# Vchitect/Latte

Measured on AMD Instinct MI355X. Metric: denoising steps/sec, higher is better.
Workload: dtype f16; 1 GPU; Latte-XL/2 FaceForensics (uncond) 16x256x256 -> latents 16x4x32x32, DDIM on the '250' respacing, random-init weights; per_gpu_batch=8, global_batch=8, parallelism=dp1 (independent samples)

## Files before the change

include/latte_amd_debug.h:

```cpp
#ifndef LATTE_AMD_DEBUG_H_
#define LATTE_AMD_DEBUG_H_
#include <stdint.h>
#ifdef __cplusplus
extern "C" {
#endif

int latte_debug_gemm(const void* A, const void* W, const float* bias, void* out, const float* gate, int M, int N,
                     int K, int gate_stride, int rows_per_sample, int epi, int dtype, int variant, void* stream);
int latte_debug_gemm_gelu(const void* A, const void* W, const float* bias, void* out, void* aux, int M, int N, int K, int epi, int dtype,
                          void* stream);
int latte_debug_gemm_lo8(const void* A, const void* W, const void* A8, const void* W8, const float* bias, void* out, const float* gate,
                         int M, int N, int K, int gate_stride, int rows_per_sample, int epi, int dtype, void* stream);
int latte_debug_pack_w8(const void* w, void* out8, int64_t n, int dtype, void* stream);
int latte_debug_pack_w4(const void* w, void* out4, void* out_scale, int N, int K, int dtype, void* stream);
int latte_debug_ln_modulate_split4(const float* x, void* y, void* y4, void* y4s, const float* shift, const float* scale, int mod_stride, int M,
                                   int D, int rows_per_sample, int dtype, void* stream);
int latte_debug_gemm_lo4(const void* A, const void* W, const void* A4, const void* A4s, const void* W4, const void* W4s, const float* bias,
                         void* out, const float* gate, int M, int N, int K, int gate_stride, int rows_per_sample, int epi, int dtype,
                         void* stream);
int latte_debug_ln_modulate_split8(const float* x, void* y, void* y8, const float* shift, const float* scale, int mod_stride, int M, int D,
                                   int rows_per_sample, int dtype, void* stream);
int latte_debug_qkv_attention_split8(const void* xn, const void* w, const float* bias, void* out, void* out8, int B, int F, int T, int D,
                                     int heads, int mode, int dtype, void* stream);
int latte_debug_gemm_choice(int M, int N, int K, int epi);
int latte_debug_qkv_attention_fusable(int D, int heads, int F, int T, int mode, int64_t rows);
int latte_debug_gemm_tn_plan(int M, int N, int K, int* rows_per_split);
int latte_debug_attention(const void* qkv, void* out, int num_seq, int L, int heads, int hd, int U,
                          int64_t sample_stride, int64_t seq_stride, int64_t row_stride, int dtype, void* stream);
int latte_debug_attention_split8(const void* qkv, void* out, void* out8, int num_seq, int L, int heads, int hd, int U, int64_t sample_stride,
                                 int64_t seq_stride, int64_t row_stride, int dtype, void* stream);
int latte_debug_qkv_attention(const void* xn, const void* w, const float* bias, void* out, void* dbg_qkv, int B, int F, int T,
                              int D, int heads, int mode, int flags, int dtype, void* stream);
int latte_debug_qkv_attention_trace(const void* xn, const void* w, const float* bias, void* out, void* dbg_qkv, long long* trace,
                                    int B, int F, int T, int D, int heads, int mode, int flags, int dtype, void* stream);
int latte_debug_attention_bwd(const void* qkv, const void* o, const void* dout, void* dqkv, float* stats, int num_seq, int L,
                              int heads, int hd, int U, int64_t sample_stride, int64_t seq_stride, int64_t row_stride, int dtype,
                              void* stream);
int latte_debug_gemm_tn(const void* dY, const void* X, float* dW, float* workspace, int64_t workspace_floats, int M, int N, int K,
                        int dtype, void* stream);
int latte_debug_gemm_tn_colsum(const void* dY, const void* X, float* dW, float* colsum, float* workspace, int64_t workspace_floats,
                               int M, int N, int K, int dtype, void* stream);
int latte_debug_ln_modulate(float* x, void* y, const float* shift, const float* scale, int mod_stride, int M, int D,
                            int rows_per_sample, const float* temp_embed, int T, int F, int dtype, void* stream);
int latte_debug_convert(const float* in, void* out, int64_t n, int dtype, void* stream);
int latte_debug_gated_add_ln(const float* x_in, const void* y, const float* gate, int gate_stride, float* x_out, void* xn,
                             const float* shift, const float* scale, int mod_stride, int M, int D, int rows_per_sample,
                             const float* temp_embed, int T, int F, int dtype, void* stream);
int latte_debug_ln_bwd(const void* dy, const float* x, const float* scale, int mod_stride, const float* dx_in, float* dx_out,
                       float* dshift, float* dscale, int out_stride, int M, int D, int rows_per_sample, const void* y2,
                       const float* gate2, int gate2_stride, void* dy2, float* gpartial, float* workspace, int64_t workspace_floats,
                       int dtype, void* stream);
int latte_debug_gate_bwd(const float* dx, const void* y, const float* gate, int gate_stride, void* dy, float* partial,
                         int64_t partial_floats, float* dgate, int out_stride, int M, int D, int rows_per_sample, int bias_partial,
                         int dtype, void* stream);
int latte_debug_loss_grad(const struct latte_schedule* s, int loss_type, const float* x_start, const float* x_t, const float* noise,
                          const float* model_out, const int64_t* t, int batch, int frames, int channels, int hw, float* dmodel_out,
                          void* stream);
int latte_debug_fill_normal(float* out, int64_t n, uint64_t seed, uint64_t offset, void* stream);
int latte_debug_tr16_probe(uint16_t* out, void* stream);

int latte_debug_conv3x3(const void* in, const float* w, const float* bias, const void* res, void* out, int N, int H, int W,
                        int Cin, int Cout, int ups, int dtype, void* stream);
int latte_debug_groupnorm(const void* x, void* y, const float* gamma, const float* beta, int N, int HW, int C, int silu,
                          int dtype, void* stream);

int latte_debug_conv3rows_f32(const void* in, const void* w_packed, const float* bias, const float* res32, float* out32, int T, int HW,
                              int Cin, int Cout, int dtype, void* stream);
// ... 37 lines not shown
```

latte_amd/_lib.py:

```python
import ctypes
import os

import torch

_HERE = os.path.dirname(os.path.abspath(__file__))
LIB_PATH = os.path.join(_HERE, "lib", "liblatte_amd.so")

c_int, c_i64, c_f32, c_void, c_char = ctypes.c_int, ctypes.c_int64, ctypes.c_float, ctypes.c_void_p, ctypes.c_char_p
c_u64 = ctypes.c_uint64


class LatteError(RuntimeError):
    pass


class ModelConfig(ctypes.Structure):
    _fields_ = [(n, c_int) for n in ("input_size", "patch_size", "in_channels", "hidden_size", "depth", "num_heads",
                                     "mlp_hidden", "num_frames", "num_classes", "learn_sigma", "extras",
                                     "compute_dtype")]


class T2VConfig(ctypes.Structure):
    _fields_ = [(n, c_int) for n in ("num_attention_heads", "attention_head_dim", "in_channels", "out_channels", "num_layers",
                                     "sample_size", "patch_size", "cross_attention_dim", "caption_channels", "video_length",
# ... 111 lines not shown
                                     c_int, c_int, c_void]),
    "latte_debug_pack_w8": (c_int, [c_void, c_void, c_i64, c_int, c_void]),
    "latte_debug_ln_modulate_split8": (c_int, [c_void, c_void, c_void, c_void, c_void, c_int, c_int, c_int, c_int, c_int, c_void]),
    "latte_debug_qkv_attention_split8": (c_int, [c_void, c_void, c_void, c_void, c_void, c_int, c_int, c_int, c_int, c_int, c_int, c_int,
                                                 c_void]),
    "latte_debug_gemm": (c_int, [c_void, c_void, c_void, c_void, c_void, c_int, c_int, c_int, c_int, c_int, c_int,
                                 c_int, c_int, c_void]),
    "latte_debug_gemm_gelu": (c_int, [c_void, c_void, c_void, c_void, c_void, c_int, c_int, c_int, c_int, c_int, c_void]),
    "latte_debug_gemm_choice": (c_int, [c_int, c_int, c_int, c_int]),
    "latte_debug_qkv_attention_fusable": (c_int, [c_int, c_int, c_int, c_int, c_int, c_i64]),
    "latte_debug_gemm_tn_plan": (c_int, [c_int, c_int, c_int, ctypes.POINTER(c_int)]),
    "latte_debug_attention": (c_int, [c_void, c_void, c_int, c_int, c_int, c_int, c_int, c_i64, c_i64, c_i64, c_int,
                                      c_void]),
    "latte_debug_qkv_attention": (c_int, [c_void, c_void, c_void, c_void, c_void, c_int, c_int, c_int, c_int, c_int, c_int, c_int,
                                          c_int, c_void]),
    "latte_debug_qkv_attention_trace": (c_int, [c_void, c_void, c_void, c_void, c_void, c_void, c_int, c_int, c_int, c_int, c_int,
                                                c_int, c_int, c_int, c_void]),
    "latte_debug_attention_bwd": (c_int, [c_void, c_void, c_void, c_void, c_void, c_int, c_int, c_int, c_int, c_int, c_i64, c_i64, c_i64,
                                          c_int, c_void]),
    "latte_debug_gemm_tn": (c_int, [c_void, c_void, c_void, c_void, c_i64, c_int, c_int, c_int, c_int, c_void]),
    "latte_debug_gemm_tn_colsum": (c_int, [c_void, c_void, c_void, c_void, c_void, c_i64, c_int, c_int, c_int, c_int, c_void]),
    "latte_debug_ln_modulate": (c_int, [c_void, c_void, c_void, c_void, c_int, c_int, c_int, c_int, c_void, c_int,
                                        c_int, c_int, c_void]),
    "latte_debug_convert": (c_int, [c_void, c_void, c_i64, c_int, c_void]),
    "latte_debug_gated_add_ln": (c_int, [c_void, c_void, c_void, c_int, c_void, c_void, c_void, c_void, c_int, c_int, c_int, c_int,
                                         c_void, c_int, c_int, c_int, c_void]),
    "latte_debug_ln_bwd": (c_int, [c_void, c_void, c_void, c_int, c_void, c_void, c_void, c_void, c_int, c_int, c_int, c_int, c_void,
                                   c_void, c_int, c_void, c_void, c_void, c_i64, c_int, c_void]),
    "latte_debug_gate_bwd": (c_int, [c_void, c_void, c_void, c_int, c_void, c_void, c_i64, c_void, c_int, c_int, c_int, c_int, c_int,
                                     c_int, c_void]),
    "latte_debug_loss_grad": (c_int, [c_void, c_int, c_void, c_void, c_void, c_void, c_void, c_int, c_int, c_int, c_int, c_void,
                                      c_void]),
    "latte_debug_fill_normal": (c_int, [c_void, c_i64, c_u64, c_u64, c_void]),
    "latte_debug_tr16_probe": (c_int, [c_void, c_void]),
    "latte_debug_set_choice": (c_int, [c_char, c_int]),
    "latte_debug_dma_probe": (c_int, [c_void, c_void, c_int, c_int, c_int, c_void]),
    "latte_debug_conv3x3": (c_int, [c_void, c_void, c_void, c_void, c_void, c_int, c_int, c_int, c_int, c_int, c_int, c_int,
                                    c_void]),
    "latte_debug_vae_trace": (c_int, [c_void, c_void, c_int, c_f32, c_int, c_void, c_void, c_void, c_void]),
    "latte_debug_vae_encode_trace": (c_int, [c_void, c_void, c_int, c_int, c_int, c_void, c_void, c_void, c_void]),
    "latte_debug_conv3x3_down_f32": (c_int, [c_void, c_void, c_void, c_void, c_void, c_int, c_int, c_int, c_int, c_int, c_int, c_void]),
    "latte_debug_vae_enc_conv_in": (c_int, [c_void, c_int, c_void, c_void, c_void, c_int, c_int, c_int, c_void]),
    "latte_debug_vae_enc_tail": (c_int, [c_void, c_void, c_void, c_void, c_void, c_void, c_void, c_int, c_int, c_int, c_void]),
    "latte_debug_conv3rows_f32": (c_int, [c_void, c_void, c_void, c_void, c_void, c_int, c_int, c_int, c_int, c_int, c_void]),
    "latte_debug_conv3x3_f32": (c_int, [c_void, c_void, c_void, c_void, c_void, c_int, c_int, c_int, c_int, c_int, c_int, c_int,
                                        c_void]),
# ... 46 lines not shown
```

latte_amd/csrc/common.h:

```cpp
#pragma once
#include <hip/hip_runtime.h>
#include <stdint.h>
#include <atomic>
#include <string>
#include <vector>

#include "../../include/latte_amd.h"

struct latte_schedule {
  int num_timesteps = 0;
  std::vector<int64_t> timestep_map;
  std::vector<double> betas, alphas_cumprod, alphas_cumprod_prev, sqrt_recip_alphas_cumprod,
      sqrt_recipm1_alphas_cumprod, posterior_variance, posterior_log_variance_clipped, posterior_mean_coef1,
      posterior_mean_coef2, log_betas, sqrt_alphas_cumprod, sqrt_one_minus_alphas_cumprod;
  int mean_type = 0;
  int var_type = 0;
  mutable float* dev_tables = nullptr;
  mutable int dev_tables_device = -1;
};
enum DevTable : int { DT_SQRT_AC = 0, DT_SQRT_1MAC, DT_COEF1, DT_COEF2, DT_POST_LOGVAR, DT_LOG_BETAS, DT_SQRT_RECIP, DT_SQRT_RECIPM1,
                      DT_FIXED_LOGVAR, LATTE_NUM_DEV_TABLES };

extern "C" int schedule_device_tables(const latte_schedule_t* s, const float** out, hipStream_t st);

// ... 107 lines not shown
  int B, F, T, D, heads, hd;
  int mode;
  float scale;
  int flags;
  int out_split;
  unsigned char* out8;
};
bool qkv_attention_fusable(int D, int heads, int hd, int F, int T, int mode, int64_t rows);
int launch_qkv_attention(const QkvAttnArgs& a, int dtype, hipStream_t st);

int launch_ln_modulate_split4(const float* x_in, half_t* y, unsigned char* y4, unsigned char* y4s, const float* shift, const float* scale,
                              int mod_stride, int M, int D, int rows_per_sample, int dtype, hipStream_t st);
int launch_ln_modulate(const float* x_in, float* x_rw, half_t* y, const float* shift, const float* scale,
                       int mod_stride, int M, int D, int rows_per_sample, const float* temp_embed, int T,
                       int F, int dtype, hipStream_t st, int split = 0,
                       unsigned char* y8 = nullptr);
int launch_pack_w8(const half_t* in, unsigned char* out, int64_t n, int dtype, hipStream_t st);
enum SmallIn : int { IN_PLAIN = 0, IN_SILU = 1, IN_TFREQ = 2 };
int launch_small_linear(int in_mode, const float* in, const int64_t* t, const float* W, const float* bias,
                        const float* add_table, const int64_t* add_idx, float* out, int B, int N, int K,
                        int out_stride, hipStream_t st);
int launch_patch_embed(const float* x, const float* Wt , const float* bias, const float* pos,
                       float* out, int BF, int C, int H, int p, int D, hipStream_t st);
int launch_final_layer(const float* x, const float* shift, const float* scale, int mod_stride,
                       const float* Wt , const float* bias, float* out, int M, int D,
                       int rows_per_sample, int T, int p, int Cout, int H, hipStream_t st);
int launch_cond_rows(const float* temb, const float* ytab, const int64_t* y, float* out, int n_steps, int bu, int D,
                     hipStream_t st);
int launch_text_proj(const float* text, const float* W, const float* bias, float* out, int B, int N, int K, hipStream_t st);
int launch_iota(int64_t* p, int n, hipStream_t st);
int launch_gated_split_reduce(float* x, const float* ws, int splits, size_t stride, const float* bias, const float* gate,
                              int gate_stride, int rows_per_sample, int M, int N, hipStream_t st);
int launch_silu_rows(const float* in, float* out, size_t n, hipStream_t st);
int launch_adaln_single(const float* tables , const float* head_table , const float* t6 ,
                        const float* temb , float* mod, int B, int nblk, int D, hipStream_t st);
int launch_permute_cf(const float* in, float* out, int B, int C, int F, int hw, int to_bfc, hipStream_t st);
int launch_fill_f32(float* p, float v, size_t n, hipStream_t st);
enum DebugChoice { DBG_ATTN_VARIANT = 0, DBG_XATTN_FLASH, DBG_TN_KERNEL, DBG_TN_WN, DBG_ATTN_BWD_TILES, DBG_CONV_KERNEL, DBG_VAE_SPLIT, DBG_NUM_CHOICES };
int debug_choice(DebugChoice c);
int set_debug_choice(const char* name, int value);

int launch_scale_f32(float* p, float s, size_t n, hipStream_t st);
int launch_scale_f32_dev(float* p, const float* s_dev, int inverse, size_t n, hipStream_t st);
int launch_t2v_guided_ddim(float* x, const float* model_out, int b, int C, int Cout, int F, int hw, float scale, float c1, float c2,
                           float c3, float c4, hipStream_t st);
int launch_mask_bias(const float* mask, float* bias, size_t n, hipStream_t st);
// ... 138 lines not shown
```

latte_amd/csrc/debug.hip:

```cpp
#include "../../include/latte_amd_debug.h"
#include "common.h"

namespace {
typedef __attribute__((ext_vector_type(4))) __bf16 bf16x4;
__global__ void tr16_probe_kernel(uint16_t* out) {
  __shared__ __attribute__((aligned(16))) uint16_t lds[512];
  for (int i = threadIdx.x; i < 512; i += 64) lds[i] = (uint16_t)i;
  __syncthreads();
  const int lane = threadIdx.x;
  auto p = (__attribute__((address_space(3))) bf16x4*)((__attribute__((address_space(3))) char*)lds + 8 * lane);
  bf16x4 v = __builtin_amdgcn_ds_read_tr16_b64_v4bf16(p);
  typedef __attribute__((ext_vector_type(4))) unsigned short u16x4;
  u16x4 u = __builtin_bit_cast(u16x4, v);
  for (int j = 0; j < 4; ++j) out[lane * 4 + j] = u[j];
}

typedef __attribute__((address_space(3))) void lds_void_t;
__global__ void __launch_bounds__(512) dma_probe_kernel(const char* src, long long* out, int mode, int reps) {
  extern __shared__ __attribute__((aligned(16))) char smem[];
  const int lane = threadIdx.x & 63, wave = __builtin_amdgcn_readfirstlane(threadIdx.x >> 6);
  const __amdgpu_buffer_rsrc_t rs = __builtin_amdgcn_make_buffer_rsrc((void*)src, 0, 1u << 30, 0x00020000);
  char* my = smem + wave * 16384;
  const unsigned base = ((blockIdx.x & 63) * 8 + wave) * 16384u;
  long long t_issue = 0, t_all = 0;
// ... 236 lines not shown
  if ((int64_t)splits * N * K > workspace_floats) return fail(LATTE_ERR_INVALID, "gemm_tn: workspace too small");
  if (int rc = launch_gemm_tn((const half_t*)dY, (const half_t*)X, workspace, M, N, K, chunk, dtype, (hipStream_t)stream)) return rc;
  return launch_split_reduce(workspace, splits, (size_t)N * K, (size_t)N * K, dW, 0, (hipStream_t)stream);
}

int latte_debug_gemm_tn_colsum(const void* dY, const void* X, float* dW, float* colsum, float* workspace, int64_t workspace_floats, int M,
                               int N, int K, int dtype, void* stream) {
  int chunk = 0;
  const int splits = gemm_tn_plan(M, N, K, &chunk);
  if (!gemm_tn8_ok(M, N, K)) return fail(LATTE_ERR_INVALID, "gemm_tn_colsum: the column sums ride on the 8-wave kernel only (M % 64, N % 128, K % 128)");
  if ((int64_t)splits * ((int64_t)N * K + N) > workspace_floats) return fail(LATTE_ERR_INVALID, "gemm_tn_colsum: workspace too small");
  float* cs = workspace + (size_t)splits * N * K;
  if (int rc = launch_gemm_tn((const half_t*)dY, (const half_t*)X, workspace, M, N, K, chunk, dtype, (hipStream_t)stream, cs)) return rc;
  if (int rc = launch_split_reduce(workspace, splits, (size_t)N * K, (size_t)N * K, dW, 0, (hipStream_t)stream)) return rc;
  return launch_split_reduce(cs, splits, (size_t)N, (size_t)N, colsum, 0, (hipStream_t)stream);
}

int latte_debug_ln_modulate(float* x, void* y, const float* shift, const float* scale, int mod_stride, int M, int D,
                            int rows_per_sample, const float* temp_embed, int T, int F, int dtype, void* stream) {
  return launch_ln_modulate(x, x, (half_t*)y, shift, scale, mod_stride, M, D, rows_per_sample, temp_embed, T, F, dtype,
                            (hipStream_t)stream);
}

int latte_debug_gated_add_ln(const float* x_in, const void* y, const float* gate, int gate_stride, float* x_out, void* xn,
                             const float* shift, const float* scale, int mod_stride, int M, int D, int rows_per_sample,
                             const float* temp_embed, int T, int F, int dtype, void* stream) {
  if (M <= 0 || rows_per_sample <= 0 || M % rows_per_sample || (temp_embed && (T <= 0 || F <= 0)))
    return fail(LATTE_ERR_INVALID, "gated_add_ln: need whole samples (M % rows_per_sample == 0) and T, F > 0 with temp_embed");
  return launch_gated_add_ln(x_in, (const half_t*)y, gate, gate_stride, x_out, (half_t*)xn, shift, scale, mod_stride, M, D,
                             rows_per_sample, temp_embed, T, F, dtype, (hipStream_t)stream);
}

static int64_t train_partial_floats(int M, int D, int rps, int nsum) {
  return (int64_t)(M / (4 * train_rows_per_run(rps))) * nsum * D;
}

int latte_debug_ln_bwd(const void* dy, const float* x, const float* scale, int mod_stride, const float* dx_in, float* dx_out,
                       float* dshift, float* dscale, int out_stride, int M, int D, int rows_per_sample, const void* y2,
                       const float* gate2, int gate2_stride, void* dy2, float* gpartial, float* workspace, int64_t workspace_floats,
                       int dtype, void* stream) {
  if (M <= 0 || rows_per_sample <= 0 || M % rows_per_sample || D <= 0)
    return fail(LATTE_ERR_INVALID, "ln_bwd: need whole samples (M % rows_per_sample == 0)");
  if (!dshift != !dscale) return fail(LATTE_ERR_INVALID, "ln_bwd: dshift and dscale are finalized together");
  if (train_partial_floats(M, D, rows_per_sample, 2) > workspace_floats) return fail(LATTE_ERR_INVALID, "ln_bwd: workspace too small");
  return launch_ln_bwd((const half_t*)dy, x, scale, mod_stride, dx_in, dx_out, workspace, dshift, dscale, out_stride, M, D,
                       rows_per_sample, dtype, (hipStream_t)stream, (const half_t*)y2, gate2, gate2_stride, (half_t*)dy2, gpartial);
// ... 160 lines not shown
```

latte_amd/csrc/engine.cpp:

```cpp
#include <algorithm>
#include <cmath>
#include <cstdio>
#include <cstring>
#include <map>
#include <string>
#include <vector>

#include "common.h"

namespace latte {

static thread_local std::string g_last_error;
static std::atomic<int> g_debug_choice[DBG_NUM_CHOICES];
int debug_choice(DebugChoice c) { return g_debug_choice[c].load(std::memory_order_relaxed); }
int set_debug_choice(const char* name, int value) {
  static const char* const names[DBG_NUM_CHOICES] = {"attn_variant", "xattn_flash", "tn_kernel", "tn_wn", "attn_bwd_tiles", "conv_kernel", "vae_split"};
  static const int allowed[DBG_NUM_CHOICES][4] = {{1, 5, 12, 13}, {1, 0, 0, 0}, {4, 0, 0, 0}, {4, 0, 0, 0}, {1, 2, 0, 0}, {1, 2, 3, 4}, {0, 0, 0, 0}};
  for (int i = 0; i < DBG_NUM_CHOICES; ++i) {
    if (name && std::string(name) == names[i]) {
      bool ok = value == 0;
      for (int k = 0; k < 4; ++k) ok = ok || (allowed[i][k] != 0 && value == allowed[i][k]);
      ok = ok || (i == DBG_VAE_SPLIT && (value >> 24) == 1);
#ifdef LATTE_GEMM_ABLATE
      ok = ok || (i == DBG_ATTN_VARIANT && value >= 7 && value <= 19);
// ... 207 lines not shown
  tm.mark(C_NONE);
  const float* modp = e->mod;
  int mstride = e->nmod;
  if (mod_override) {
    modp = mod_override;
    mstride = mod_stride_override;
  } else {
    if ((rc = launch_small_linear(IN_TFREQ, nullptr, t, e->t0_w, e->t0_b, nullptr, nullptr, e->temb0, B, D, 256, D, st))) return rc;
    const float* add_tab = c.extras == 2 ? e->ytab : c.extras == 78 ? e->txt_proj : nullptr;
    const int64_t* add_idx = c.extras == 78 ? e->iota : y;
    if ((rc = launch_small_linear(IN_SILU, e->temb0, nullptr, e->t2_w, e->t2_b, add_tab, add_idx, e->cvec, B, D, D, D, st))) return rc;
    if ((rc = launch_silu_rows(e->cvec, e->cvec, (size_t)B * D, st))) return rc;
    if ((rc = launch_small_linear(IN_PLAIN, e->cvec, nullptr, e->ada_w, e->ada_b, nullptr, nullptr, e->mod, B, e->nmod, D,
                                  e->nmod, st))) return rc;
    if (c.extras == 78) {
      const size_t fo = (size_t)c.depth * 6 * D;
      if ((rc = launch_small_linear(IN_SILU, e->temb0, nullptr, e->t2_w, e->t2_b, nullptr, nullptr, e->cvec_t, B, D, D, D, st))) return rc;
      if ((rc = launch_silu_rows(e->cvec_t, e->cvec_t, (size_t)B * D, st))) return rc;
      if ((rc = launch_small_linear(IN_PLAIN, e->cvec_t, nullptr, e->ada_w + fo * D, e->ada_b + fo, nullptr, nullptr,
                                    e->mod + fo, B, 2 * D, D, e->nmod, st))) return rc;
    }
  }
  tm.mark(C_COND);
  if (cfg_dup) {
    const int hb = B / 2;
    if ((rc = launch_patch_embed(x, e->pe_wt, e->pe_b, e->pos, e->xres, hb * F, e->Cin, e->H, c.patch_size, D, st))) return rc;
    if ((rc = launch_patch_embed(x, e->pe_wt, e->pe_b, e->pos, e->xres + (size_t)hb * rps * D, hb * F, e->Cin, e->H,
                                 c.patch_size, D, st))) return rc;
  } else {
    if ((rc = launch_patch_embed(x, e->pe_wt, e->pe_b, e->pos, e->xres, B * F, e->Cin, e->H, c.patch_size, D, st))) return rc;
  }
  tm.mark(C_PATCH);
  int gsplit = cfg_dup ? e->guided_split : 0;
  if (dt != LATTE_DTYPE_F16) gsplit &= 3;
  if ((gsplit & 16) && !gemm_lo4_ok(M, e->Hm, D)) gsplit = (gsplit & ~16) | 8;
  if (gsplit & 16) gsplit &= ~10;
  if (gsplit & 4) gsplit &= ~1;
  if (gsplit & 8) gsplit &= ~2;
  if ((gsplit & 4) && !gemm_lo8_ok(M, D, D)) gsplit = (gsplit & ~4) | 1;
  if ((gsplit & 8) && !gemm_lo8_ok(M, e->Hm, D)) gsplit = (gsplit & ~8) | 2;
  if ((gsplit & 3) && (uint64_t)e->rows_pad * 2 * D * 2 >= (1ull << 32)) gsplit &= ~3;
  if (gsplit) gsplit = ensure_split_weights(e, gsplit, st);
  int gactive = gsplit & 26;

  for (int i = 0; i < c.depth; ++i) {
    const bool spatial = (i % 2) == 0;
    const BlockW& w = e->blocks[i];
    const float* mb = modp + (size_t)i * 6 * D;
    bool split_proj = false;
    const float* te = (i == 1) ? e->temp : nullptr;
    if ((rc = launch_ln_modulate(e->xres, e->xres, e->xn, mb, mb + D, mstride, M, D, rps, te, T, F, dt, st))) return rc;
    tm.mark(C_LN);
    GemmArgs g{};
    g.M = M; g.rows_per_sample = rps; g.gate_stride = mstride;
    const half_t* attn_out = e->xn;
    if (((e->fuse_qkv_attn >> (spatial ? 0 : 1)) & 1) && qkv_attention_fusable(D, c.num_heads, e->hd, F, T, spatial ? 0 : 1, M)) {
      QkvAttnArgs qa{};
      qa.xn = e->xn; qa.w = w.qkv_w; qa.bias = w.qkv_b; qa.out = e->qkv; qa.B = B; qa.F = F; qa.T = T; qa.D = D;
      qa.heads = c.num_heads; qa.hd = e->hd; qa.mode = spatial ? 0 : 1; qa.scale = 1.0f / std::sqrt((float)e->hd);
      qa.flags = ((e->fuse_qkv_attn >> 2) & 7) ^ 7;
      split_proj = gsplit & 5;
      qa.out_split = (gsplit & 4) ? 2 : (gsplit & 1);
      qa.out8 = e->lo8;
      gactive |= gsplit & 5;
      if ((rc = launch_qkv_attention(qa, dt, st))) return rc;
      tm.mark(spatial ? C_QKVATTN_S : C_QKVATTN_T);
      attn_out = e->qkv;
    } else {
      g.A = e->xn; g.W = w.qkv_w; g.bias = w.qkv_b; g.out = e->qkv; g.N = 3 * D; g.K = D;
      if ((rc = launch_gemm(g, EPI_BIAS_H16, dt, e->gemm_variant_of[0] ? e->gemm_variant_of[0] : e->gemm_variant, st))) return rc;
      tm.mark(C_QKV);
      AttnArgs a{};
      a.qkv = e->qkv; a.out = e->xn; a.heads = c.num_heads; a.hd = e->hd; a.D = D;
      a.sample_stride = rps; a.scale = 1.0f / std::sqrt((float)e->hd);
      if (spatial) { a.num_seq = B * F; a.L = T; a.U = F; a.seq_stride = T; a.row_stride = 1; }
// ... 688 lines not shown
```

latte_amd/csrc/pointwise.hip:

```cpp
#include "common.h"
#include "mfma_util.h"

namespace latte {
namespace {

template <int NCH, int DT, bool ADD_TE, int SPLIT = 0>
__global__ void __launch_bounds__(256) ln_modulate_kernel(const float* __restrict__ x_in, float* x_rw,
                                                          half_t* __restrict__ y, const float* __restrict__ shift,
                                                          const float* __restrict__ scale, int mod_stride, int M,
                                                          int rows_per_sample, const float* __restrict__ te, int T,
                                                          int F, unsigned char* __restrict__ y8 = nullptr,
                                                          unsigned char* __restrict__ y4s = nullptr) {
  constexpr int D = NCH * 128;
  constexpr int NT = NCH * 32;
  constexpr int NQ = (NT + 63) / 64;
  const int lane = threadIdx.x & 63;
  const int row = blockIdx.x * 4 + (threadIdx.x >> 6);
  if (row >= M) return;
  const float4* xr = (const float4*)(x_in + (size_t)row * D);
  auto has = [&](int c) -> bool { return (c + 1) * 64 <= NT || c * 64 + lane < NT; };
  float4 v[NQ];
#pragma unroll
  for (int c = 0; c < NQ; ++c) v[c] = has(c) ? xr[c * 64 + lane] : make_float4(0.f, 0.f, 0.f, 0.f);
  const int smp = row / rows_per_sample;
// ... 227 lines not shown
      s += v[c].x + v[c].y;
    }
    const float mean = wave_sum(s) * (1.0f / D);
    float q = 0.f;
#pragma unroll
    for (int c = 0; c < NCH; ++c) {
      const float a = v[c].x - mean, b = v[c].y - mean;
      q += a * a + b * b;
    }
    const float rstd = 1.0f / sqrtf(wave_sum(q) * (1.0f / D) + 1e-6f);
    const int smp = row / rows_per_sample;
    const float2* sh = (const float2*)(shift + (size_t)smp * mod_stride);
    const float2* sc = (const float2*)(scale + (size_t)smp * mod_stride);
#pragma unroll
    for (int c = 0; c < NCH; ++c) {
      const float2 a = sh[c * 64 + lane], b = sc[c * 64 + lane];
      xo[c * 64 + lane] = make_float2((v[c].x - mean) * rstd * (1.0f + b.x) + a.x,
                                      (v[c].y - mean) * rstd * (1.0f + b.y) + a.y);
    }
  }
  __syncthreads();
  const int P = p * p * Cout;
  const int G = H / p;
  if (P == 32) {
    const int j = lane & 31, ksl = wave * 2 + (lane >> 5);
    constexpr int KSL = D / 8;
    float acc[FL_ROWS];
#pragma unroll
    for (int r = 0; r < FL_ROWS; ++r) acc[r] = 0.f;
    for (int k = ksl * KSL; k < (ksl + 1) * KSL; k += 4) {
      const float w0 = Wt[(size_t)k * 32 + j], w1 = Wt[(size_t)(k + 1) * 32 + j], w2 = Wt[(size_t)(k + 2) * 32 + j],
                  w3 = Wt[(size_t)(k + 3) * 32 + j];
#pragma unroll
      for (int r = 0; r < FL_ROWS; ++r) {
        const float4 xv = *(const float4*)(xs + r * D + k);
        acc[r] = fmaf(xv.w, w3, fmaf(xv.z, w2, fmaf(xv.y, w1, fmaf(xv.x, w0, acc[r]))));
      }
    }
#pragma unroll
    for (int r = 0; r < FL_ROWS; ++r) acc[r] += __shfl_xor(acc[r], 32, 64);
    __syncthreads();
    if (lane < 32) {
#pragma unroll
      for (int r = 0; r < FL_ROWS; ++r) xs[(wave * FL_ROWS + r) * 32 + j] = acc[r];
    }
    __syncthreads();
    const int rr = threadIdx.x >> 5, jj = threadIdx.x & 31;
    const int row = row0 + rr;
    if (row < M) {
      const float r = ((xs[(0 * FL_ROWS + rr) * 32 + jj] + xs[(1 * FL_ROWS + rr) * 32 + jj]) +
                       (xs[(2 * FL_ROWS + rr) * 32 + jj] + xs[(3 * FL_ROWS + rr) * 32 + jj])) + bias[jj];
      const int c = jj % Cout, qi = (jj / Cout) % p, pi = jj / (Cout * p);
      const int bf = row / T, tt = row % T;
      const int hp = tt / G, wp = tt % G;
      out[(((size_t)bf * Cout + c) * H + hp * p + pi) * H + wp * p + qi] = r;
    }
    return;
  }
  for (int idx = threadIdx.x; idx < FL_ROWS * P; idx += 256) {
    const int rr = idx / P, j = idx % P;
    const int row = row0 + rr;
    if (row >= M) continue;
    const float* xr = xs + rr * D;
    float a0 = 0.f, a1 = 0.f, a2 = 0.f, a3 = 0.f;
    for (int k = 0; k < D; k += 4) {
      a0 = fmaf(xr[k + 0], Wt[(size_t)(k + 0) * P + j], a0);
      a1 = fmaf(xr[k + 1], Wt[(size_t)(k + 1) * P + j], a1);
      a2 = fmaf(xr[k + 2], Wt[(size_t)(k + 2) * P + j], a2);
      a3 = fmaf(xr[k + 3], Wt[(size_t)(k + 3) * P + j], a3);
    }
    const float r = (a0 + a1) + (a2 + a3) + bias[j];
    const int c = j % Cout, qi = (j / Cout) % p, pi = j / (Cout * p);
    const int bf = row / T, tt = row % T;
    const int hp = tt / G, wp = tt % G;
    out[(((size_t)bf * Cout + c) * H + hp * p + pi) * H + wp * p + qi] = r;
  }
}

__global__ void cond_rows_kernel(const float* __restrict__ temb, const float* __restrict__ ytab, const int64_t* __restrict__ y,
                                 float* __restrict__ out, int n_steps, int bu, int D) {
  const size_t total = (size_t)n_steps * bu * D;
  for (size_t i = (size_t)blockIdx.x * blockDim.x + threadIdx.x; i < total; i += (size_t)gridDim.x * blockDim.x) {
    const int d = (int)(i % D);
    const size_t r = i / D;
    const int b = (int)(r % bu), step = (int)(r / bu);
    float v = temb[(size_t)step * D + d];
    if (ytab != nullptr) v += ytab[(size_t)y[b] * D + d];
    out[i] = silu(v);
  }
}

constexpr int TP_B = 8;
__global__ void __launch_bounds__(256) text_proj_kernel(const float* __restrict__ text, const float* __restrict__ W,
                                                        const float* __restrict__ bias, float* __restrict__ out, int B,
                                                        int N, int K) {
  const int lane = threadIdx.x & 63;
  const int n = blockIdx.x * 4 + (threadIdx.x >> 6);
  if (n >= N) return;
// ... 554 lines not shown
      break;
    case IN_SILU:
      hipLaunchKernelGGL(small_linear_kernel<IN_SILU>, grid, block, 0, st, in, t, W, bias, add_table, add_idx, out, B, N, K, out_stride);
      break;
    case IN_TFREQ:
      hipLaunchKernelGGL(small_linear_kernel<IN_TFREQ>, grid, block, 0, st, in, t, W, bias, add_table, add_idx, out, B, N, K, out_stride);
      break;
    default:
      return fail(LATTE_ERR_INVALID, "small_linear: bad input mode");
  }
  LATTE_HIP(hipGetLastError());
  return LATTE_OK;
}

int launch_patch_embed(const float* x, const float* Wt, const float* bias, const float* pos, float* out, int BF,
                       int C, int H, int p, int D, hipStream_t st) {
  const int G = H / p, ntok = BF * G * G, K = C * p * p;
  dim3 grid((ntok + PE_TOK - 1) / PE_TOK, D / 128), block(128);
  hipLaunchKernelGGL(patch_embed_kernel, grid, block, PE_TOK * K * sizeof(float), st, x, Wt, bias, pos, out, ntok, C, H, p, D);
  LATTE_HIP(hipGetLastError());
  return LATTE_OK;
}

int launch_final_layer(const float* x, const float* shift, const float* scale, int mod_stride, const float* Wt,
                       const float* bias, float* out, int M, int D, int rows_per_sample, int T, int p, int Cout,
                       int H, hipStream_t st) {
  dim3 grid((M + FL_ROWS - 1) / FL_ROWS), block(256);
  const size_t lds = (size_t)FL_ROWS * D * sizeof(float);
#define FL_LAUNCH(NCH)                                                                                       \
  hipLaunchKernelGGL(final_layer_kernel<NCH>, grid, block, lds, st, x, shift, scale, mod_stride, Wt, bias, out, M, \
                     rows_per_sample, T, p, Cout, H)
  LATTE_NCH_SWITCH(D, FL_LAUNCH)
#undef FL_LAUNCH
  LATTE_HIP(hipGetLastError());
  return LATTE_OK;
}

int launch_cond_rows(const float* temb, const float* ytab, const int64_t* y, float* out, int n_steps, int bu, int D,
                     hipStream_t st) {
  const size_t n = (size_t)n_steps * bu * D;
  hipLaunchKernelGGL(cond_rows_kernel, dim3(grid_for(n, 256)), dim3(256), 0, st, temb, ytab, y, out, n_steps, bu, D);
  LATTE_HIP(hipGetLastError());
  return LATTE_OK;
}

int launch_text_proj(const float* text, const float* W, const float* bias, float* out, int B, int N, int K,
                     hipStream_t st) {
  if (K % 128) return fail(LATTE_ERR_INVALID, "text_proj: K must be a multiple of 128");
  hipLaunchKernelGGL(text_proj_kernel, dim3((N + 3) / 4), dim3(256), 0, st, text, W, bias, out, B, N, K);
// ... 145 lines not shown
```

Measured before the change: 264.5 sample-steps/s.

## Fuse patch embed with first LN-modulate and add persistent final-layer kernel

Adds a persistent patch_embed_ln kernel that computes the patch embedding, adds bias and position embedding, writes the residual, and applies the first block's LayerNorm modulation in one pass. The engine then skips the separate ln_modulate launch for block 0. The final layer gets a new persistent kernel for p*p*Cout==32, with the weight held in padded LDS and the reduction done by wave shuffles, replacing the old in-kernel P==32 branch. Both kernels run once per denoising step, so any gain is small relative to 28 transformer blocks. The fused path also handles the CFG-duplicate case through src_tok indexing.

```diff
diff --git a/include/latte_amd_debug.h b/include/latte_amd_debug.h
--- a/include/latte_amd_debug.h
+++ b/include/latte_amd_debug.h
@@ -43,6 +43,13 @@
 int latte_debug_ln_modulate(float* x, void* y, const float* shift, const float* scale, int mod_stride, int M, int D,
                             int rows_per_sample, const float* temp_embed, int T, int F, int dtype, void* stream);
 int latte_debug_convert(const float* in, void* out, int64_t n, int dtype, void* stream);
+int latte_debug_patch_embed(const float* x, const float* wt, const float* bias, const float* pos, float* out, int BF, int C, int H, int p,
+                            int D, void* stream);
+int latte_debug_patch_embed_ln(const float* x, const float* wt, const float* bias, const float* pos, float* xout, void* xn,
+                               const float* shift, const float* scale, int mod_stride, int M, int src_tok, int rows_per_sample, int C,
+                               int H, int p, int D, int dtype, void* stream);
+int latte_debug_final_layer(const float* x, const float* shift, const float* scale, int mod_stride, const float* wt, const float* bias,
+                            float* out, int M, int D, int rows_per_sample, int T, int p, int Cout, int H, void* stream);
 int latte_debug_gated_add_ln(const float* x_in, const void* y, const float* gate, int gate_stride, float* x_out, void* xn,
                              const float* shift, const float* scale, int mod_stride, int M, int D, int rows_per_sample,
                              const float* temp_embed, int T, int F, int dtype, void* stream);
diff --git a/latte_amd/_lib.py b/latte_amd/_lib.py
--- a/latte_amd/_lib.py
+++ b/latte_amd/_lib.py
@@ -157,6 +157,11 @@
     "latte_debug_gemm_tn_colsum": (c_int, [c_void, c_void, c_void, c_void, c_void, c_i64, c_int, c_int, c_int, c_int, c_void]),
     "latte_debug_ln_modulate": (c_int, [c_void, c_void, c_void, c_void, c_int, c_int, c_int, c_int, c_void, c_int,
                                         c_int, c_int, c_void]),
+    "latte_debug_patch_embed": (c_int, [c_void, c_void, c_void, c_void, c_void, c_int, c_int, c_int, c_int, c_int, c_void]),
+    "latte_debug_patch_embed_ln": (c_int, [c_void, c_void, c_void, c_void, c_void, c_void, c_void, c_void, c_int, c_int, c_int, c_int,
+                                           c_int, c_int, c_int, c_int, c_int, c_void]),
+    "latte_debug_final_layer": (c_int, [c_void, c_void, c_void, c_int, c_void, c_void, c_void, c_int, c_int, c_int, c_int, c_int, c_int,
+                                        c_int, c_void]),
     "latte_debug_convert": (c_int, [c_void, c_void, c_i64, c_int, c_void]),
     "latte_debug_gated_add_ln": (c_int, [c_void, c_void, c_void, c_int, c_void, c_void, c_void, c_void, c_int, c_int, c_int, c_int,
                                          c_void, c_int, c_int, c_int, c_void]),
diff --git a/latte_amd/csrc/common.h b/latte_amd/csrc/common.h
--- a/latte_amd/csrc/common.h
+++ b/latte_amd/csrc/common.h
@@ -153,6 +153,10 @@
                         int out_stride, hipStream_t st);
 int launch_patch_embed(const float* x, const float* Wt , const float* bias, const float* pos,
                        float* out, int BF, int C, int H, int p, int D, hipStream_t st);
+bool patch_embed_ln_fusable(int C, int p, int D);
+int launch_patch_embed_ln(const float* x, const float* Wt , const float* bias, const float* pos, float* xout, half_t* xn,
+                          const float* shift, const float* scale, int mod_stride, int M, int src_tok, int rows_per_sample, int C, int H,
+                          int p, int D, int dtype, hipStream_t st);
 int launch_final_layer(const float* x, const float* shift, const float* scale, int mod_stride,
                        const float* Wt , const float* bias, float* out, int M, int D,
                        int rows_per_sample, int T, int p, int Cout, int H, hipStream_t st);
diff --git a/latte_amd/csrc/debug.hip b/latte_amd/csrc/debug.hip
--- a/latte_amd/csrc/debug.hip
+++ b/latte_amd/csrc/debug.hip
@@ -282,6 +282,26 @@
                             (hipStream_t)stream);
 }
 
+int latte_debug_patch_embed(const float* x, const float* wt, const float* bias, const float* pos, float* out, int BF, int C, int H, int p,
+                            int D, void* stream) {
+  if (BF <= 0 || C <= 0 || p <= 0 || H <= 0 || H % p || D % 128) return fail(LATTE_ERR_INVALID, "patch_embed: bad shape");
+  return launch_patch_embed(x, wt, bias, pos, out, BF, C, H, p, D, (hipStream_t)stream);
+}
+
+int latte_debug_patch_embed_ln(const float* x, const float* wt, const float* bias, const float* pos, float* xout, void* xn,
+                               const float* shift, const float* scale, int mod_stride, int M, int src_tok, int rows_per_sample, int C,
+                               int H, int p, int D, int dtype, void* stream) {
+  return launch_patch_embed_ln(x, wt, bias, pos, xout, (half_t*)xn, shift, scale, mod_stride, M, src_tok, rows_per_sample, C, H, p, D,
+                               dtype, (hipStream_t)stream);
+}
+
+int latte_debug_final_layer(const float* x, const float* shift, const float* scale, int mod_stride, const float* wt, const float* bias,
+                            float* out, int M, int D, int rows_per_sample, int T, int p, int Cout, int H, void* stream) {
+  if (M <= 0 || rows_per_sample <= 0 || T <= 0 || p <= 0 || Cout <= 0 || H % p || (H / p) * (H / p) != T || M % T)
+    return fail(LATTE_ERR_INVALID, "final_layer: bad shape");
+  return launch_final_layer(x, shift, scale, mod_stride, wt, bias, out, M, D, rows_per_sample, T, p, Cout, H, (hipStream_t)stream);
+}
+
 int latte_debug_gated_add_ln(const float* x_in, const void* y, const float* gate, int gate_stride, float* x_out, void* xn,
                              const float* shift, const float* scale, int mod_stride, int M, int D, int rows_per_sample,
                              const float* temp_embed, int T, int F, int dtype, void* stream) {
diff --git a/latte_amd/csrc/engine.cpp b/latte_amd/csrc/engine.cpp
--- a/latte_amd/csrc/engine.cpp
+++ b/latte_amd/csrc/engine.cpp
@@ -253,7 +253,12 @@
     }
   }
   tm.mark(C_COND);
-  if (cfg_dup) {
+  const bool fused_embed = patch_embed_ln_fusable(e->Cin, c.patch_size, D);
+  if (fused_embed) {
+    const int src_tok = (cfg_dup ? B / 2 : B) * rps;
+    if ((rc = launch_patch_embed_ln(x, e->pe_wt, e->pe_b, e->pos, e->xres, e->xn, modp, modp + D, mstride, M, src_tok, rps, e->Cin,
+                                    e->H, c.patch_size, D, dt, st))) return rc;
+  } else if (cfg_dup) {
     const int hb = B / 2;
     if ((rc = launch_patch_embed(x, e->pe_wt, e->pe_b, e->pos, e->xres, hb * F, e->Cin, e->H, c.patch_size, D, st))) return rc;
     if ((rc = launch_patch_embed(x, e->pe_wt, e->pe_b, e->pos, e->xres + (size_t)hb * rps * D, hb * F, e->Cin, e->H,
@@ -280,8 +285,10 @@
     const float* mb = modp + (size_t)i * 6 * D;
     bool split_proj = false;
     const float* te = (i == 1) ? e->temp : nullptr;
-    if ((rc = launch_ln_modulate(e->xres, e->xres, e->xn, mb, mb + D, mstride, M, D, rps, te, T, F, dt, st))) return rc;
-    tm.mark(C_LN);
+    if (i > 0 || !fused_embed) {
+      if ((rc = launch_ln_modulate(e->xres, e->xres, e->xn, mb, mb + D, mstride, M, D, rps, te, T, F, dt, st))) return rc;
+      tm.mark(C_LN);
+    }
     GemmArgs g{};
     g.M = M; g.rows_per_sample = rps; g.gate_stride = mstride;
     const half_t* attn_out = e->xn;
diff --git a/latte_amd/csrc/pointwise.hip b/latte_amd/csrc/pointwise.hip
--- a/latte_amd/csrc/pointwise.hip
+++ b/latte_amd/csrc/pointwise.hip
@@ -273,41 +273,6 @@
   __syncthreads();
   const int P = p * p * Cout;
   const int G = H / p;
-  if (P == 32) {
-    const int j = lane & 31, ksl = wave * 2 + (lane >> 5);
-    constexpr int KSL = D / 8;
-    float acc[FL_ROWS];
-#pragma unroll
-    for (int r = 0; r < FL_ROWS; ++r) acc[r] = 0.f;
-    for (int k = ksl * KSL; k < (ksl + 1) * KSL; k += 4) {
-      const float w0 = Wt[(size_t)k * 32 + j], w1 = Wt[(size_t)(k + 1) * 32 + j], w2 = Wt[(size_t)(k + 2) * 32 + j],
-                  w3 = Wt[(size_t)(k + 3) * 32 + j];
-#pragma unroll
-      for (int r = 0; r < FL_ROWS; ++r) {
-        const float4 xv = *(const float4*)(xs + r * D + k);
-        acc[r] = fmaf(xv.w, w3, fmaf(xv.z, w2, fmaf(xv.y, w1, fmaf(xv.x, w0, acc[r]))));
-      }
-    }
-#pragma unroll
-    for (int r = 0; r < FL_ROWS; ++r) acc[r] += __shfl_xor(acc[r], 32, 64);
-    __syncthreads();
-    if (lane < 32) {
-#pragma unroll
-      for (int r = 0; r < FL_ROWS; ++r) xs[(wave * FL_ROWS + r) * 32 + j] = acc[r];
-    }
-    __syncthreads();
-    const int rr = threadIdx.x >> 5, jj = threadIdx.x & 31;
-    const int row = row0 + rr;
-    if (row < M) {
-      const float r = ((xs[(0 * FL_ROWS + rr) * 32 + jj] + xs[(1 * FL_ROWS + rr) * 32 + jj]) +
-                       (xs[(2 * FL_ROWS + rr) * 32 + jj] + xs[(3 * FL_ROWS + rr) * 32 + jj])) + bias[jj];
-      const int c = jj % Cout, qi = (jj / Cout) % p, pi = jj / (Cout * p);
-      const int bf = row / T, tt = row % T;
-      const int hp = tt / G, wp = tt % G;
-      out[(((size_t)bf * Cout + c) * H + hp * p + pi) * H + wp * p + qi] = r;
-    }
-    return;
-  }
   for (int idx = threadIdx.x; idx < FL_ROWS * P; idx += 256) {
     const int rr = idx / P, j = idx % P;
     const int row = row0 + rr;
@@ -325,6 +290,220 @@
     const int bf = row / T, tt = row % T;
     const int hp = tt / G, wp = tt % G;
     out[(((size_t)bf * Cout + c) * H + hp * p + pi) * H + wp * p + qi] = r;
+  }
+}
+
+constexpr int PEL_K = 16, PEL_THREADS = 768;
+template <int NCH, int DT>
+__global__ void __launch_bounds__(PEL_THREADS) patch_embed_ln_kernel(const float* __restrict__ x, const float* __restrict__ Wt,
+                                                                      const float* __restrict__ bias, const float* __restrict__ pos,
+                                                                      float* __restrict__ xout, half_t* __restrict__ y,
+                                                                      const float* __restrict__ shift, const float* __restrict__ scale,
+                                                                      int mod_stride, int M, int src_tok, int rows_per_sample, int C,
+                                                                      int H, int p) {
+  constexpr int D = NCH * 128;
+  constexpr int NT = NCH * 32;
+  constexpr int NQ = (NT + 63) / 64;
+  extern __shared__ float4 pel_w[];
+  for (int i = threadIdx.x; i < PEL_K * NT; i += PEL_THREADS) pel_w[i] = ((const float4*)Wt)[i];
+  __syncthreads();
+  const int lane = threadIdx.x & 63;
+  const int G = H / p, T = G * G;
+  auto has = [&](int c) -> bool { return (c + 1) * 64 <= NT || c * 64 + lane < NT; };
+  int ch[NQ];
+#pragma unroll
+  for (int c = 0; c < NQ; ++c) ch[c] = has(c) ? c * 64 + lane : NT - 1;
+  int xoff[PEL_K];
+#pragma unroll
+  for (int k = 0; k < PEL_K; ++k) xoff[k] = ((k / (p * p)) * H + (k / p) % p) * H + k % p;
+  const int nwaves = gridDim.x * (PEL_THREADS / 64);
+  const int wave0 = __builtin_amdgcn_readfirstlane(blockIdx.x * (PEL_THREADS / 64) + (threadIdx.x >> 6));
+  for (int row = wave0; row < M; row += nwaves) {
+    float xv[PEL_K];
+    {
+      const int n = row % src_tok;
+      const int bf = n / T, tt = n % T;
+      const int hp = tt / G, wp = tt % G;
+      const float* xp = x + ((size_t)bf * C * H + hp * p) * H + wp * p;
+#pragma unroll
+      for (int k = 0; k < PEL_K; ++k) xv[k] = xp[xoff[k]];
+    }
+    float4 v[NQ];
+#pragma unroll
+    for (int c = 0; c < NQ; ++c) {
+      v[c] = make_float4(0.f, 0.f, 0.f, 0.f);
+#pragma unroll
+      for (int k = 0; k < PEL_K; ++k) {
+        if (k % 4 == 0) __builtin_amdgcn_sched_barrier(0);
+        const float4 w = pel_w[k * NT + ch[c]];
+        v[c].x = fmaf(xv[k], w.x, v[c].x);
+        v[c].y = fmaf(xv[k], w.y, v[c].y);
+        v[c].z = fmaf(xv[k], w.z, v[c].z);
+        v[c].w = fmaf(xv[k], w.w, v[c].w);
+      }
+    }
+    __builtin_amdgcn_sched_barrier(0);
+    const float4* pr = (const float4*)(pos + (size_t)(row % T) * D);
+    float4* xw = (float4*)(xout + (size_t)row * D);
+    const int smp = row / rows_per_sample;
+    const float4* sh = (const float4*)(shift + (size_t)smp * mod_stride);
+    const float4* sc = (const float4*)(scale + (size_t)smp * mod_stride);
+    float4 sha[NQ], sca[NQ];
+#pragma unroll
+    for (int c = 0; c < NQ; ++c) {
+      const float4 bv = ((const float4*)bias)[ch[c]], pv = pr[ch[c]];
+      sha[c] = sh[ch[c]];
+      sca[c] = sc[ch[c]];
+      v[c] = make_float4(v[c].x + bv.x + pv.x, v[c].y + bv.y + pv.y, v[c].z + bv.z + pv.z, v[c].w + bv.w + pv.w);
+      if (has(c)) xw[c * 64 + lane] = v[c];
+      else v[c] = make_float4(0.f, 0.f, 0.f, 0.f);
+    }
+    float s = 0.f;
+#pragma unroll
+    for (int c = 0; c < NQ; ++c) s += (v[c].x + v[c].y) + (v[c].z + v[c].w);
+    const float mean = wave_sum(s) * (1.0f / D);
+    float q = 0.f;
+#pragma unroll
+    for (int c = 0; c < NQ; ++c) {
+      const float a = v[c].x - mean, b = v[c].y - mean, d = v[c].z - mean, e = v[c].w - mean;
+      const float t = (a * a + b * b) + (d * d + e * e);
+      q += has(c) ? t : 0.f;
+    }
+    const float rstd = 1.0f / sqrtf(wave_sum(q) * (1.0f / D) + 1e-6f);
+    u32x2* yr = (u32x2*)(y + (size_t)row * D);
+#pragma unroll
+    for (int c = 0; c < NQ; ++c) {
+      const float4 a = sha[c], b = sca[c];
+      const float o0 = (v[c].x - mean) * rstd * (1.0f + b.x) + a.x;
+      const float o1 = (v[c].y - mean) * rstd * (1.0f + b.y) + a.y;
+      const float o2 = (v[c].z - mean) * rstd * (1.0f + b.z) + a.z;
+      const float o3 = (v[c].w - mean) * rstd * (1.0f + b.w) + a.w;
+      if (has(c)) yr[c * 64 + lane] = (u32x2){pack2<DT>(o0, o1), pack2<DT>(o2, o3)};
+    }
+  }
+}
+
+constexpr int FLP_THREADS = 512;
+template <int N, int MASK, int LEN>
+__device__ __forceinline__ void fold_halves(float (&a)[LEN], int lane) {
+  const bool up = (lane & MASK) != 0;
+#pragma unroll
+  for (int i = 0; i < N; ++i) {
+    const float keep = up ? a[i + N] : a[i], send = up ? a[i] : a[i + N];
+    a[i] = keep + __shfl_xor(send, MASK, 64);
+  }
+}
+template <int NCH>
+__global__ void __launch_bounds__(FLP_THREADS) final_layer_p32_kernel(const float* __restrict__ x, const float* __restrict__ shift,
+                                                                       const float* __restrict__ scale, int mod_stride,
+                                                                       const float* __restrict__ Wt, const float* __restrict__ bias,
+                                                                       float* __restrict__ out, int M, int rows_per_sample, int T,
+                                                                       int p, int Cout, int H) {
+  constexpr int D = NCH * 128;
+  constexpr int NT = NCH * 32;
+  constexpr int NQ = (NT + 63) / 64;
+  extern __shared__ float4 flp_w[];
+  for (int i = threadIdx.x; i < D * 8; i += FLP_THREADS) flp_w[(i >> 5) * 33 + (i & 31)] = ((const float4*)Wt)[i];
+  __syncthreads();
+  const int lane = threadIdx.x & 63;
+  auto has = [&](int c) -> bool { return (c + 1) * 64 <= NT || c * 64 + lane < NT; };
+  const int nwaves = gridDim.x * (FLP_THREADS / 64);
+  const int wave0 = __builtin_amdgcn_readfirstlane(blockIdx.x * (FLP_THREADS / 64) + (threadIdx.x >> 6));
+  const int G = H / p;
+  const int j = (lane & 1) * 16 + ((lane >> 1) & 15);
+  const float bj = bias[j];
+  const int oc = j % Cout, oq = (j / Cout) % p, op = j / (Cout * p);
+  for (int row0 = wave0 * 2; row0 < M; row0 += nwaves * 2) {
+    float4 xn[2][NQ];
+#pragma unroll
+    for (int r = 0; r < 2; ++r) {
+      const int row = min(row0 + r, M - 1);
+      if (r) __builtin_amdgcn_sched_barrier(0);
+      const float4* xr = (const float4*)(x + (size_t)row * D);
+      float4 v[NQ];
+#pragma unroll
+      for (int c = 0; c < NQ; ++c) v[c] = has(c) ? xr[c * 64 + lane] : make_float4(0.f, 0.f, 0.f, 0.f);
+      const int smp = row / rows_per_sample;
+      const float4* sh = (const float4*)(shift + (size_t)smp * mod_stride);
+      const float4* sc = (const float4*)(scale + (size_t)smp * mod_stride);
+      float4 sha[NQ], sca[NQ];
+#pragma unroll
+      for (int c = 0; c < NQ; ++c) {
+        sha[c] = has(c) ? sh[c * 64 + lane] : make_float4(0.f, 0.f, 0.f, 0.f);
+        sca[c] = has(c) ? sc[c * 64 + lane] : make_float4(0.f, 0.f, 0.f, 0.f);
+      }
+      float s = 0.f;
+#pragma unroll
+      for (int c = 0; c < NQ; ++c) s += (v[c].x + v[c].y) + (v[c].z + v[c].w);
+      const float mean = wave_sum(s) * (1.0f / D);
+      float q = 0.f;
+#pragma unroll
+      for (int c = 0; c < NQ; ++c) {
+        if (has(c)) {
+          const float a = v[c].x - mean, b = v[c].y - mean, d = v[c].z - mean, e = v[c].w - mean;
+          q += (a * a + b * b) + (d * d + e * e);
+        }
+      }
+      const float rstd = 1.0f / sqrtf(wave_sum(q) * (1.0f / D) + 1e-6f);
+#pragma unroll
+      for (int c = 0; c < NQ; ++c) {
+        const float4 a = sha[c], b = sca[c];
+        xn[r][c] = has(c) ? make_float4((v[c].x - mean) * rstd * (1.0f + b.x) + a.x, (v[c].y - mean) * rstd * (1.0f + b.y) + a.y,
+                                        (v[c].z - mean) * rstd * (1.0f + b.z) + a.z, (v[c].w - mean) * rstd * (1.0f + b.w) + a.w)
+                          : make_float4(0.f, 0.f, 0.f, 0.f);
+      }
+    }
+    float part[4];
+#pragma unroll
+    for (int h = 0; h < 2; ++h) {
+      float acc[2][16];
+#pragma unroll
+      for (int r = 0; r < 2; ++r)
+#pragma unroll
+        for (int i = 0; i < 16; ++i) acc[r][i] = 0.f;
+#pragma unroll
+      for (int c = 0; c < NQ; ++c) {
+        if (has(c)) {
+          const int kq = c * 64 + lane;
+#pragma unroll
+          for (int u = 0; u < 4; ++u) {
+            const float x0 = u == 0 ? xn[0][c].x : u == 1 ? xn[0][c].y : u == 2 ? xn[0][c].z : xn[0][c].w;
+            const float x1 = u == 0 ? xn[1][c].x : u == 1 ? xn[1][c].y : u == 2 ? xn[1][c].z : xn[1][c].w;
+            if ((u & 1) == 0) __builtin_amdgcn_sched_barrier(0);
+#pragma unroll
+            for (int j4 = 0; j4 < 4; ++j4) {
+              const float4 w = flp_w[kq * 33 + u * 8 + h * 4 + j4];
+              acc[0][4 * j4 + 0] = fmaf(x0, w.x, acc[0][4 * j4 + 0]);
+              acc[0][4 * j4 + 1] = fmaf(x0, w.y, acc[0][4 * j4 + 1]);
+              acc[0][4 * j4 + 2] = fmaf(x0, w.z, acc[0][4 * j4 + 2]);
+              acc[0][4 * j4 + 3] = fmaf(x0, w.w, acc[0][4 * j4 + 3]);
+              acc[1][4 * j4 + 0] = fmaf(x1, w.x, acc[1][4 * j4 + 0]);
+              acc[1][4 * j4 + 1] = fmaf(x1, w.y, acc[1][4 * j4 + 1]);
+              acc[1][4 * j4 + 2] = fmaf(x1, w.z, acc[1][4 * j4 + 2]);
+              acc[1][4 * j4 + 3] = fmaf(x1, w.w, acc[1][4 * j4 + 3]);
+            }
+          }
+        }
+      }
+      __builtin_amdgcn_sched_barrier(0);
+#pragma unroll
+      for (int r = 0; r < 2; ++r) {
+        fold_halves<8, 16>(acc[r], lane);
+        fold_halves<4, 8>(acc[r], lane);
+        fold_halves<2, 4>(acc[r], lane);
+        fold_halves<1, 2>(acc[r], lane);
+        part[2 * r + h] = acc[r][0];
+      }
+    }
+    fold_halves<2, 32>(part, lane);
+    fold_halves<1, 1>(part, lane);
+    const float res = part[0] + bj;
+    const int row = row0 + (lane >> 5);
+    if (row < M) {
+      const int bf = row / T, tt = row % T;
+      const int hp = tt / G, wp = tt % G;
+      out[(((size_t)bf * Cout + oc) * H + hp * p + op) * H + wp * p + oq] = res;
+    }
   }
 }
 
@@ -925,9 +1104,85 @@
   return LATTE_OK;
 }
 
+static int device_cus(int* out) {
+  int dev = 0;
+  LATTE_HIP(hipGetDevice(&dev));
+  static std::atomic<int> cus[64];
+  int n = cus[dev & 63].load(std::memory_order_relaxed);
+  if (n <= 0) {
+    LATTE_HIP(hipDeviceGetAttribute(&n, hipDeviceAttributeMultiprocessorCount, dev));
+    if (n <= 0) return fail(LATTE_ERR_HIP, "device reports no compute units");
+    cus[dev & 63].store(n, std::memory_order_relaxed);
+  }
+  *out = n;
+  return LATTE_OK;
+}
+
+static int resident_grid(const void* fn, int threads, int lds, int cus, int want, unsigned int* out) {
+  int per_cu = 0;
+  LATTE_HIP(hipOccupancyMaxActiveBlocksPerMultiprocessor(&per_cu, fn, threads, (size_t)lds));
+  const int fit = (per_cu > 0 ? per_cu : 1) * cus;
+  *out = (unsigned int)(want < fit ? want : fit);
+  return LATTE_OK;
+}
+
+bool patch_embed_ln_fusable(int C, int p, int D) { return C * p * p == PEL_K && D % 128 == 0 && D / 128 <= 9 && D / 128 != 5 && D / 128 != 7; }
+
+int launch_patch_embed_ln(const float* x, const float* Wt, const float* bias, const float* pos, float* xout, half_t* xn,
+                          const float* shift, const float* scale, int mod_stride, int M, int src_tok, int rows_per_sample, int C, int H,
+                          int p, int D, int dtype, hipStream_t st) {
+  if (!patch_embed_ln_fusable(C, p, D) || M <= 0 || src_tok <= 0 || rows_per_sample <= 0 || H % p)
+    return fail(LATTE_ERR_INVALID, "patch_embed_ln: need C p p == 16, D = 128*{1,2,3,4,6,8,9} and positive row counts");
+  int cus = 0;
+  if (int rc = device_cus(&cus)) return rc;
+  const int lds = PEL_K * D * (int)sizeof(float);
+  constexpr int WAVES = PEL_THREADS / 64;
+  const int want = (M + WAVES - 1) / WAVES;
+  dim3 grid(1), block(PEL_THREADS);
+#define PEL_LAUNCH(NCH)                                                                                                          \
+  do {                                                                                                                           \
+    static std::atomic<uint64_t> done[2];                                                                                        \
+    if (dtype == LATTE_DTYPE_BF16) {                                                                                             \
+      if (int rc = ensure_dynamic_lds((const void*)patch_embed_ln_kernel<NCH, LATTE_DTYPE_BF16>, lds, done[0])) return rc;       \
+      if (int rc = resident_grid((const void*)patch_embed_ln_kernel<NCH, LATTE_DTYPE_BF16>, PEL_THREADS, lds, cus, want, &grid.x)) return rc; \
+      hipLaunchKernelGGL((patch_embed_ln_kernel<NCH, LATTE_DTYPE_BF16>), grid, block, lds, st, x, Wt, bias, pos, xout, xn, shift, \
+                         scale, mod_stride, M, src_tok, rows_per_sample, C, H, p);                                               \
+    } else {                                                                                                                     \
+      if (int rc = ensure_dynamic_lds((const void*)patch_embed_ln_kernel<NCH, LATTE_DTYPE_F16>, lds, done[1])) return rc;        \
+      if (int rc = resident_grid((const void*)patch_embed_ln_kernel<NCH, LATTE_DTYPE_F16>, PEL_THREADS, lds, cus, want, &grid.x)) return rc; \
+      hipLaunchKernelGGL((patch_embed_ln_kernel<NCH, LATTE_DTYPE_F16>), grid, block, lds, st, x, Wt, bias, pos, xout, xn, shift,  \
+                         scale, mod_stride, M, src_tok, rows_per_sample, C, H, p);                                               \
+    }                                                                                                                            \
+  } while (0)
+  LATTE_NCH_SWITCH(D, PEL_LAUNCH)
+#undef PEL_LAUNCH
+  LATTE_HIP(hipGetLastError());
+  return LATTE_OK;
+}
+
 int launch_final_layer(const float* x, const float* shift, const float* scale, int mod_stride, const float* Wt,
                        const float* bias, float* out, int M, int D, int rows_per_sample, int T, int p, int Cout,
                        int H, hipStream_t st) {
+  if (p * p * Cout == 32) {
+    int cus = 0;
+    if (int rc = device_cus(&cus)) return rc;
+    const int lds = (D / 4) * 33 * 16;
+    constexpr int WAVES = FLP_THREADS / 64;
+    const int want = (M + 2 * WAVES - 1) / (2 * WAVES);
+    dim3 grid(1), block(FLP_THREADS);
+#define FLP_LAUNCH(NCH)                                                                                                      \
+  do {                                                                                                                       \
+    static std::atomic<uint64_t> done{0};                                                                                    \
+    if (int rc = ensure_dynamic_lds((const void*)final_layer_p32_kernel<NCH>, lds, done)) return rc;                         \
+    if (int rc = resident_grid((const void*)final_layer_p32_kernel<NCH>, FLP_THREADS, lds, cus, want, &grid.x)) return rc;   \
+    hipLaunchKernelGGL(final_layer_p32_kernel<NCH>, grid, block, lds, st, x, shift, scale, mod_stride, Wt, bias, out, M,     \
+                       rows_per_sample, T, p, Cout, H);                                                                      \
+  } while (0)
+    LATTE_NCH_SWITCH(D, FLP_LAUNCH)
+#undef FLP_LAUNCH
+    LATTE_HIP(hipGetLastError());
+    return LATTE_OK;
+  }
   dim3 grid((M + FL_ROWS - 1) / FL_ROWS), block(256);
   const size_t lds = (size_t)FL_ROWS * D * sizeof(float);
 #define FL_LAUNCH(NCH)                                                                                       \
```

Result: no change. 265.0 sample-steps/s, median of 6 (+0.2%).
